# ClickHouse/libhdfs3

Measured on AMD Instinct MI355X. Metric: device-resident CRC32C GiB/s over 512 B HDFS chunks; % of HBM roofline, higher is better.
Workload: dtype u8

## Files before the change

libhdfs3_amd/csrc/crc32c_experiments.hip:

```cpp
#include "crc32c_wave.h"

namespace hdfs3crc {
namespace {

template <int BPC, bool V>
hipError_t launch_exp(const LaunchEnv &env, int variant, const ChunkLaunch &a) {
    const auto [tab, fold, grid_cap, s] = std::tie(env.tables, env.fold, env.grid_cap, env.stream);
    if constexpr (BPC > kRoundBytes) {
        if (variant == 115) return launch_r3<BPC, V, 1, true, true>(a, tab, fold, grid_cap, s);
        if (variant == 123) return launch_r3<BPC, V, 1, true>(a, tab, fold, grid_cap, s);
    }
    if constexpr (BPC <= kRoundBytes) {
        switch (variant) {
        case 92:
            return launch_wave3<BPC, V, false, true, kLabEarly>(a, tab, fold, grid_cap, s);
        case 93:
            return launch_wave3<BPC, V, false, false>(a, tab, fold, grid_cap, s);
        case 94:
            return launch_wave3<BPC, V, false, V>(a, tab, fold, grid_cap, s);
        case 95:
            return launch_wave3<BPC, V, false, true, kLabNoHold>(a, tab, fold, grid_cap, s);
        case 77:
            return launch_wave3<BPC, V, false, true, kLabNoMath>(a, tab, fold, grid_cap, s);
        case 99:
        case 100: {
            const uint64_t units = a.len / kRoundBytes;
            const uint64_t npk = variant == 99 ? 1 : 8;
            const uint64_t upp = units / npk;
            if (a.len % kRoundBytes || units % npk || (upp & (upp - 1)) || a.chunk_base) return hipErrorInvalidValue;
            ChunkLaunch p = a;
            p.npk = npk;
            p.pitch = upp * kRoundBytes;
            p.crc_pitch = upp * (kRoundBytes / BPC) * 4;
            p.last_len = uint32_t(upp * kRoundBytes);
            if (!packet_geom(p.pitch, p.last_len, npk, BPC, &p.geom)) return hipErrorInvalidValue;
            return launch_wave3<BPC, V, true, false>(p, tab, fold, grid_cap, s);
        }
        case 115:
            return launch_wave3<BPC, V, false, true, kLabPrio>(a, tab, fold, grid_cap, s);
        case 117:
            return launch_wave3<BPC, V, false, true, kLabNoPrio>(a, tab, fold, grid_cap, s);
        case 118:
            return launch_wave3<BPC, V, false, true, kLabNoStore>(a, tab, fold, grid_cap, s);
        case 119:
            return launch_wave3<BPC, V, false, true, kLabNearStore>(a, tab, fold, grid_cap, s);
        case 123:
            return launch_wave3<BPC, V, false, true>(a, tab, fold, grid_cap, s);
        case 122:
            return launch_wave3<BPC, V, false, true, kLabNoStage>(a, tab, fold, grid_cap, s);
        case 130:
            return launch_wave3<BPC, V, false, true, kLabStageWin>(a, tab, fold, grid_cap, s);
        case 157:
            return launch_wave3<BPC, V, false, true, kLabFull16>(a, tab, fold, grid_cap, s);
        case 128:
            return launch_wave3<BPC, V, false, true, kLabStorePlain>(a, tab, fold, grid_cap, s);
        case 146:
            return launch_wave3<BPC, V, false, true, kLabClock | kLabMid>(a, tab, fold, grid_cap, s);
        case 147:
            return launch_wave3<BPC, V, false, true, kLabNoTabLoad | kLabClock | kLabMid>(a, tab, fold, grid_cap, s);
        case 148:
            return launch_wave3<BPC, V, false, true, kLabNoTabLoad>(a, tab, fold, grid_cap, s);
        case 137:
            return launch_wave3<BPC, V, false, true, kLabWg1024>(a, tab, fold, grid_cap, s);
        case 162:
            return launch_wave3<BPC, V, false, true, kLabOneRound>(a, tab, fold, grid_cap, s);
        case 132:
            return launch_wave3<BPC, V, false, true, 0, 256>(a, tab, fold, grid_cap, s);
        case 134:
            return launch_wave3<BPC, V, false, true, 0, 512>(a, tab, fold, grid_cap, s);
        case 125:
            return launch_wave3<BPC, V, false, true, kLabClock>(a, tab, fold, grid_cap, s);
        case 78:
            return launch_wave3<BPC, V, false, true, kLabNoMath | kLabNoFill>(a, tab, fold, grid_cap, s);
        default: return hipErrorInvalidValue;
        }
    }
    return hipErrorInvalidValue;
}

}

hipError_t launch_experiment(const LaunchEnv &env, int variant, const ChunkLaunch &a, bool verify) {
    return dispatch_bpc<true>(a.bpc, [&](auto bpc) {
        return verify ? launch_exp<bpc(), true>(env, variant, a) : launch_exp<bpc(), false>(env, variant, a);
    });
}

void set_variant(int v) { g_variant = v; }

hipError_t lab_clock_buffer(unsigned long long *d, unsigned int cap, unsigned int *n_out) {
    unsigned int n = 0;
    hipError_t e = hipMemcpyFromSymbol(&n, HIP_SYMBOL(g_lab_clk_n), sizeof n);
    if (e != hipSuccess) return e;
    if (n_out) *n_out = n;
    const unsigned int zero = 0;
    if ((e = hipMemcpyToSymbol(HIP_SYMBOL(g_lab_clk), &d, sizeof d)) != hipSuccess) return e;
    if ((e = hipMemcpyToSymbol(HIP_SYMBOL(g_lab_clk_cap), &cap, sizeof cap)) != hipSuccess) return e;
    return hipMemcpyToSymbol(HIP_SYMBOL(g_lab_clk_n), &zero, sizeof zero);
}

hipError_t lab_wave_buffer(unsigned long long *d, unsigned int cap, unsigned int *n_out) {
    if (n_out) *n_out = g_lab_seq.exchange(0);
    hipError_t e;
    const unsigned long long *none = nullptr;
    if ((e = hipMemcpyToSymbol(HIP_SYMBOL(g_lab_wave), &none, sizeof none)) != hipSuccess) return e;
    if (!d || !cap) return hipSuccess;
    if ((e = hipMemcpyToSymbol(HIP_SYMBOL(g_lab_wave_cap), &cap, sizeof cap)) != hipSuccess) return e;
    return hipMemcpyToSymbol(HIP_SYMBOL(g_lab_wave), &d, sizeof d);
}

hipError_t launch_stream_read(const uint8_t *d, uint64_t len, uint32_t *sink, int grid,
                              hipStream_t stream, bool overlap_previous) {
    const bool nt = grid < 0;
    const dim3 g(nt ? -grid : grid), b(256);
    auto k = nt ? stream_read_kernel<true> : stream_read_kernel<false>;
    if (overlap_previous)
        hipExtLaunchKernelGGL(k, g, b, 0, stream, nullptr, nullptr, hipExtAnyOrderLaunch, d, len / 16, sink,
                              g_lab_seq++);
    else
        hipLaunchKernelGGL(k, g, b, 0, stream, d, len / 16, sink, g_lab_seq++);
    return hipGetLastError();
}

hipError_t launch_lane_read(const uint8_t *d, uint64_t len, uint32_t bpc, uint32_t *sink,
                            int grid_cap, hipStream_t stream) {
    const int variant = int(bpc >> 16);
    bpc &= 0xFFFFu;
    const uint64_t chunks = len / bpc;
    const uint64_t lanes = variant == 2 ? chunks * 8 : variant == 3 ? chunks * 4 : chunks;
    const uint64_t need = (lanes + kBlockThreads - 1) / kBlockThreads;
    const int grid = int(need < uint64_t(grid_cap) ? need : uint64_t(grid_cap));
#define LR(B, V) hipLaunchKernelGGL((lane_read_kernel<B, V>), dim3(grid), dim3(kBlockThreads), 0, stream, d, chunks, sink)
#define LRV(B)                          \
    switch (variant) {                  \
    case 0: LR(B, 0); break;            \
    case 1: LR(B, 1); break;            \
    case 2: LR(B, 2); break;            \
    case 3: LR(B, 3); break;            \
    default: LR(B, 4); break;           \
    }
    switch (bpc) {
    case 512: LRV(512); break;
    case 2048: LRV(2048); break;
    case 4096: LRV(4096); break;
    default: return hipErrorInvalidValue;
    }
#undef LRV
#undef LR
    return hipGetLastError();
}

}
```

libhdfs3_amd/csrc/crc32c_wave.h:

```cpp
#pragma once

#include "crc32c_device.h"

namespace hdfs3crc {
namespace {

constexpr int kLabEarly = 1;
constexpr int kLabNoMath = 2;
constexpr int kLabNoHold = 4;
constexpr int kLabNoFill = 8;
constexpr int kLabPrio = 16;
constexpr int kLabNoPrio = 32;
constexpr int kLabNoStore = 64;
constexpr int kLabNearStore = 128;
constexpr int kLabNoStage = 1024;
constexpr int kLabStageWin = 2048;
constexpr int kLabClock = 4096;
constexpr int kLabStorePlain = 8192;
constexpr int kLabWg1024 = 16384;
constexpr int kLabNoTabLoad = 2097152;
constexpr int kLabFull16 = 8388608;
constexpr int kLabOneRound = 4194304;
constexpr int kLabMid = 1048576;
constexpr int kStageWords = 512;
constexpr uint32_t kStageMaxRounds(int bpc) { return uint32_t(bpc / 16); }

constexpr uint32_t kPrioMinRounds = 16;

typedef __attribute__((address_space(1))) const uint32_t gcu32;
typedef __attribute__((address_space(1))) const uint8_t gcu8;
typedef __attribute__((address_space(1))) uint8_t gu8;
typedef __attribute__((address_space(1))) uint32_t gu32;
typedef __attribute__((address_space(1))) unsigned long long gu64;
typedef __attribute__((address_space(4))) const SegLaunch CSegLaunch;
typedef __attribute__((address_space(4))) const DevSegment CDevSegment;

struct WView {
    const uint8_t *p;
    uint8_t *w;
    uint64_t key;
    uint32_t nb;
};

template <int CPU>
struct BlockWalk {
    static constexpr bool kLaneView = true;
    static constexpr bool kContiguous = true;
    const uint8_t *data;
    uint8_t *words;
    uint64_t key0, first, stride;
    uint32_t K;
    const uint8_t *dummy;
    uint32_t kq = 0, kr = 0;
    __device__ __forceinline__ WView view(uint32_t k) const {
        const uint64_t u = first + uint64_t(k) * stride;
        const bool in = k < K;
        return WView{in ? data + u * kRoundBytes : dummy, in ? words + 4 * CPU * u : const_cast<uint8_t *>(dummy),
                     key0 + CPU * u, uint32_t(kRoundBytes)};
    }
};

template <int CPU>
struct PitchWalk {
    static constexpr bool kLaneView = true;
    static constexpr bool kContiguous = false;
    const uint8_t *data;
    uint8_t *words;
    uint64_t dpitch, wpitch, first, stride;
    uint32_t K;
    uint32_t upp, magic, shift, ptail, lunits, ltail, lpk;
    const uint8_t *dummy;
    __device__ __forceinline__ WView view(uint32_t k) const {
        const uint32_t u = uint32_t(first + uint64_t(k) * stride);
        const uint32_t pk = uint32_t((uint64_t(u) * magic) >> shift), r = u - pk * upp;
        const bool lastp = pk == lpk;
        const uint32_t nb = r + 1 == (lastp ? lunits : upp) ? (lastp ? ltail : ptail) : uint32_t(kRoundBytes);
        const bool in = k < K;
        return WView{in ? data + uint64_t(pk) * dpitch + uint64_t(r) * kRoundBytes : dummy,
                     in ? words + uint64_t(pk) * wpitch + 4 * CPU * r : const_cast<uint8_t *>(dummy),
                     (uint64_t(pk) << 32) | (CPU * r), in ? nb : uint32_t(kRoundBytes)};
    }
};

template <int CPU, bool UNI>
struct SegWalk {
    static constexpr bool kLaneView = false;
    static constexpr bool kContiguous = false;
    CSegLaunch *L;
    uint64_t first, stride;
    uint32_t K;
    const uint8_t *dummy;
    uint64_t c_begin = 1, c_end = 0, c_key = 0;
    uint64_t c_wlen = 0;
    const uint8_t *c_data = nullptr;
    uint8_t *c_crc = nullptr;
    uint32_t c_si = ~0u;
    static constexpr uint32_t kBpc = uint32_t(kRoundBytes / CPU);

    __device__ __forceinline__ static uint64_t wlen(uint64_t len) { return len / kBpc * kBpc; }
    __device__ __forceinline__ static uint64_t units(uint64_t len) { return (wlen(len) + kRoundBytes - 1) / kRoundBytes; }
    __device__ __forceinline__ CDevSegment *segp(uint32_t i) const {
        return L->seg ? (CDevSegment *)(L->seg) + i : L->inl + i;
    }
    __device__ __forceinline__ uint32_t seg_of(uint64_t u) const {
        if constexpr (UNI) {
            const uint32_t si = uint32_t(u) / uint32_t(L->uniform);
            return si < L->nseg ? si : L->nseg - 1;
        } else {
            uint32_t lo = 0, hi = L->nseg - 1;
            while (lo < hi) {
                const uint32_t mid = (lo + hi + 1) >> 1;
                if (rfl64(segp(mid)->unit_begin) <= u) lo = mid;
                else hi = mid - 1;
            }
            return lo;
        }
    }
    __device__ __forceinline__ WView view(uint32_t k) {
        if (k >= K) return WView{dummy, const_cast<uint8_t *>(dummy), 0, uint32_t(kRoundBytes)};
        const uint64_t u = first + uint64_t(k) * stride;
        if (u < c_begin || u >= c_end) {
            uint32_t si;
            if constexpr (UNI) {
                si = seg_of(u);
            } else {
                const uint32_t nx = c_si + 1;
                if (nx < L->nseg && u >= rfl64(segp(nx)->unit_begin) &&
                    u < rfl64(segp(nx)->unit_begin) + units(rfl64(segp(nx)->len)))
                    si = nx;
                else if (L->unit_seg)
                    si = __builtin_amdgcn_readfirstlane(
                        ((__attribute__((address_space(4))) const uint32_t *)(L->unit_seg))[u]);
                else
                    si = seg_of(u);
            }
            if (L->stride) {
                const bool lastp = si + 1 >= L->nseg;
                c_begin = uint64_t(si) * L->uniform;
                c_wlen = wlen(lastp ? L->inl[1].len : L->inl[0].len);
                c_end = c_begin + (lastp ? units(L->inl[1].len) : L->uniform);
                c_data = L->inl[0].data + uint64_t(si) * L->stride;
                c_crc = L->dense_words ? L->dense_words + 4 * CPU * c_begin : L->inl[0].crc + uint64_t(si) * L->stride;
                c_key = uint64_t(si) << 32;
            } else {
                CDevSegment *sd = segp(si);
                c_begin = rfl64(sd->unit_begin);
                c_wlen = wlen(rfl64(sd->len));
                c_end = c_begin + (c_wlen + kRoundBytes - 1) / kRoundBytes;
                c_data = reinterpret_cast<const uint8_t *>(rfl64(reinterpret_cast<uint64_t>(sd->data)));
                c_crc = L->dense_words ? L->dense_words + 4 * CPU * c_begin
                                       : reinterpret_cast<uint8_t *>(rfl64(reinterpret_cast<uint64_t>(sd->crc)));
                c_key = rfl64(sd->key_base);
            }
            c_si = si;
        }
        const uint64_t r = u - c_begin, left = c_wlen - r * kRoundBytes;
        return WView{c_data + r * kRoundBytes, c_crc + 4 * CPU * r, c_key + CPU * r,
                     left < kRoundBytes ? uint32_t(left) : uint32_t(kRoundBytes)};
    }
};

template <int BPC, bool VERIFY, bool SOLO, bool HOLD, int LAB, int TPB, class Walk>
__device__ __forceinline__ void wave_rounds(Walk &walk, uint32_t *lds, const uint32_t *__restrict__ g_tab,
                                            const uint32_t *__restrict__ g_nib, unsigned long long *result,
                                            unsigned long long *lab_mid = nullptr) {
    constexpr int G = BPC / 64;
    constexpr bool kHalfFold = G <= 32;
    constexpr bool LATE = (LAB & kLabEarly) == 0, NOMATH = (LAB & kLabNoMath) != 0;
    constexpr bool kWrong = (LAB & (kLabNoMath | kLabNoFill | kLabNoTabLoad)) != 0;
    const uint32_t lane = threadIdx.x & 63;
    const uint32_t j = lane % G;
    const uint32_t lane_off = 64 * (lane & 15) + 16 * (lane >> 4);
    const uint32_t K = walk.K;

    constexpr int kFillIters = 1024 / TPB;
    static_assert(kFillIters * TPB == 1024, "TPB divides 1024");
    uint32_t tw[kFillIters];
    u32x4 n0[kFillIters], n1[kFillIters];
#pragma unroll
    for (int f = 0; f < kFillIters; ++f) {
        const uint32_t t = threadIdx.x + f * TPB;
        if constexpr ((LAB & kLabNoTabLoad) != 0) {
            tw[f] = t * 0x9E3779B9u;
            n0[f] = u32x4{t, t ^ 1u, t ^ 2u, t ^ 3u};
            n1[f] = n0[f];
            continue;
        }
        tw[f] = g_tab[t];
        if constexpr (kHalfFold) {
            const uint32_t fk = 2 * (t >> 8) + ((t >> 3) & 1), fe = (t >> 4) & 15, fc = 4 * (t & 7);
            n0[f] = *reinterpret_cast<const u32x4 *>(g_nib + (fk * 16 + fe) * 64 + fc);
        } else {
            n0[f] = *reinterpret_cast<const u32x4 *>(g_nib + 8 * t);
            n1[f] = *reinterpret_cast<const u32x4 *>(g_nib + 8 * t + 4);
        }
    }
    WView cv0 = walk.view(0), cv1 = walk.view(1);
    __builtin_amdgcn_sched_barrier(0);
    Round a0, a1, b0, b1;
    load_round_buf<true>(a0, cv0.p, lane_off, cv0.nb);
    load_round_buf<true>(a1, cv1.p, lane_off, cv1.nb);
    __builtin_amdgcn_sched_barrier(0);
#pragma unroll
    for (int f = 0; f < kFillIters; ++f) {
        const uint32_t tt = threadIdx.x + f * TPB, slice = tt >> 8, entry = tt & 255;
        const uint32_t slot0 = ((slice >> 1) << 16 | entry << 8 | (slice & 1) << 7) / 16;
        const uint32_t w = tw[f];
        const uint32_t byte_t = (slot0 | (tt & 7)) << 4;
#pragma unroll
        for (int r = 0; r < ((LAB & kLabNoFill) ? 0 : 8); ++r)
            *reinterpret_cast<u32x4 *>(reinterpret_cast<uint8_t *>(lds) + (byte_t ^ uint32_t(16 * r))) = u32x4{w, w, w, w};
        if constexpr (kHalfFold) {
            reinterpret_cast<u32x4 *>(lds + kHalfFoldOff / 4)[tt] = n0[f];
        } else {
            u32x4 *dst = reinterpret_cast<u32x4 *>(reinterpret_cast<uint8_t *>(lds) + kFoldLdsOff) + 2 * tt;
            dst[0] = n0[f];
            dst[1] = n1[f];
        }
    }
    lds_barrier();
    if constexpr ((LAB & kLabMid) != 0) lab_mid[0] = __builtin_amdgcn_s_memrealtime();
    const Lut t(lds);
    const NibFold nf(lds);
    auto fold = [&](uint32_t x) -> uint32_t {
        if constexpr (kHalfFold) return fold_half(reinterpret_cast<const uint8_t *>(lds), x);
        return nf.apply(x);
    };
    const uint32_t woff = 4 * (lane / G);
    const uint32_t coff = (lane / G) * BPC;
    WView pv0 = walk.view(2), pv1 = walk.view(3);

    auto wrsrc = [](const WView &v) {
        return __builtin_amdgcn_make_buffer_rsrc(v.w, 0, __builtin_amdgcn_readfirstlane(v.nb / (BPC / 4)), 0x00020000);
    };
    auto want_of = [&](const WView &v) -> uint32_t {
        if constexpr (VERIFY) return __builtin_amdgcn_raw_buffer_load_b32(wrsrc(v), woff, 0, 0);
        return 0;
    };
    constexpr bool kHold = HOLD && !VERIFY && G == 8;
    constexpr bool kAddr = !Walk::kLaneView;
    auto held_store = [&](gu8 *p, uint32_t v) { *(gu32 *)p = v; };
    uint32_t line = 0;
    uint32_t hold[kHold ? 8 : 1];
    gu32 *laddr = nullptr;
    gu32 *hold_addr[kHold && kAddr ? 8 : 1];
    uint32_t nheld = 0, hold_base = 0;
    auto flush = [&]() {
#pragma unroll
        for (int i = 0; i < (kHold ? 8 : 0); ++i) {
            if (uint32_t(i) < nheld && ((LAB & kLabNoStore) == 0 || hold[i] == 0x9E3779B9u)) {
                if constexpr ((LAB & kLabNearStore) != 0 && !kAddr) {
                    *(gu32 *)((gu8 *)walk.view(0).w + 4 * lane) = hold[i];
                } else if constexpr (kAddr) {
                    if (hold_addr[i]) *hold_addr[i] = hold[i];
                } else {
                    const uint32_t kk = 8 * (hold_base + nheld - 1 - i) + (lane >> 3);
                    if (kk < K) {
                        const WView v = walk.view(kk);
                        if ((lane & 7) * BPC < v.nb) held_store((gu8 *)v.w + 4 * (lane & 7), hold[i]);
                    }
                }
            }
        }
        hold_base += nheld;
        nheld = 0;
    };
    constexpr bool kStage = !VERIFY && (LAB & kStageWords) != 0 && Walk::kContiguous && kHalfFold && TPB == 1024;
    constexpr uint32_t kCpw = 64 / G;
    constexpr uint32_t kSR = kStageMaxRounds(BPC);
    uint32_t *stage = lds + kLdsBytesWave / 4 - 4096;
    const uint32_t slot = threadIdx.x >> 6;
    auto stage_store = [&](gu8 *p, uint32_t v) {
        if constexpr ((LAB & kLabNoStore) != 0) {
            if (v != 0x9E3779B9u) return;
        }
        if constexpr (kStage && (LAB & kLabStorePlain) == 0) {
            const uint64_t wb = rfl64(reinterpret_cast<uint64_t>(walk.words));
            const __amdgpu_buffer_rsrc_t rs = __builtin_amdgcn_make_buffer_rsrc(
                reinterpret_cast<void *>(wb), 0, 0x7FFFFFFF, 0x00020000);
            __builtin_amdgcn_raw_buffer_store_b32(v, rs, uint32_t(reinterpret_cast<uint64_t>(p) - wb), 0, 1 | 2 | 16);
        } else {
            *(gu32 *)p = v;
        }
    };
    uint32_t kq_flush = 0;
    if constexpr (kStage) kq_flush = walk.kq - (walk.kr == 0 ? 1u : 0u);
    auto stage_flush = [&](uint32_t kend) {
        if constexpr (kStage) {
            if (kend % kSR == 0 && kend <= kq_flush && walk.kq != 0) {
                lds_barrier();
                const uint64_t wg_first = walk.first - slot;
#pragma unroll
                for (int p = 0; p < 4; ++p) {
                    const uint32_t t = threadIdx.x + 1024 * p, kk = t / (16 * kCpw), s = (t / kCpw) & 15,
                                   c = t % kCpw;
                    stage_store((gu8 *)walk.words +
                                    4 * kCpw * (wg_first + s + uint64_t(kend - kSR + kk) * walk.stride) + 4 * c,
                                stage[t]);
                }
                lds_barrier();
            }
        }
    };
    constexpr bool kHold64 = !VERIFY && G == 64 && Walk::kContiguous && (LAB & kLabNoHold) == 0;
    uint32_t line64 = 0;
    auto finish = [&](uint32_t k, const WView &v, uint32_t y, uint32_t want) {
        if constexpr (kHold64) {
            if (k >= K) return;
            const uint32_t yy = __builtin_amdgcn_readfirstlane(y);
            line64 = lane == (k & 63) ? yy : line64;
            if ((k & 63) == 63 || k + 1 == K) {
                const uint32_t kk = (k & ~63u) + lane;
                if (lane <= (k & 63)) held_store((gu8 *)walk.view(kk).w, line64);
            }
            return;
        }
        if constexpr (kStage) {
            if (k < K && j == 0) stage[((k % kSR) * 16 + slot) * kCpw + lane / G] = y;
            return;
        }
        if constexpr (kHold) {
            if (k >= K) return;
            const uint32_t r = k & 7;
            const uint32_t got = uint32_t(__builtin_amdgcn_ds_bpermute(int(32 * (lane & 7)), int(y)));
            const bool mine = (lane >> 3) == r;
            line = mine ? got : line;
            if constexpr (kAddr)
                laddr = mine ? ((lane & 7) * BPC < v.nb ? (gu32 *)((gu8 *)v.w + 4 * (lane & 7)) : nullptr) : laddr;
            if (r == 7 || k + 1 == K) {
#pragma unroll
                for (int i = (kHold ? 7 : 0); i > 0; --i) {
                    hold[i] = hold[i - 1];
                    if constexpr (kAddr) hold_addr[i] = hold_addr[i - 1];
                }
                hold[0] = line;
                if constexpr (kAddr) {
                    hold_addr[0] = laddr;
                    laddr = nullptr;
                }
                if (++nheld == 8) flush();
            }
            return;
        }
        if (k >= K || j != 0) return;
        const uint32_t c = y;
        if constexpr (VERIFY) {
            if ((want != c) != kWrong && coff < v.nb)
                __hip_atomic_fetch_max((gu64 *)result, ~(unsigned long long)(v.key + lane / G), __ATOMIC_RELAXED,
                                       __HIP_MEMORY_SCOPE_AGENT);
        } else {
            __builtin_amdgcn_raw_buffer_store_b32(c, wrsrc(v), woff, 0, 0);
        }
    };
    auto word = [](const Round &r, int i) -> uint32_t { return r.w[i >> 2][i & 3]; };
    auto look = [&](uint32_t x) -> Look {
        if constexpr (NOMATH) return Look{{x, 0u, 0u, 0u}};
        return lookups(t, x);
    };
    auto chains = [&](Round &c0, Round &c1, uint32_t &x0, uint32_t &x1) {
        x0 = word(c0, 0);
        x1 = word(c1, 0);
        Look l0 = look(x0), l1;
        __builtin_amdgcn_sched_barrier(0);
        if constexpr ((LAB & kLabFull16) != 0) {
#pragma unroll
            for (int i = 0; i < 16; ++i) {
                l1 = look(x1);
                __builtin_amdgcn_sched_barrier(0);
                x0 = combine(l0, i < 15 ? word(c0, i < 15 ? i + 1 : 15) : 0u);
                __builtin_amdgcn_sched_barrier(0);
                if (i < 15) l0 = look(x0);
                __builtin_amdgcn_sched_barrier(0);
                x1 = combine(l1, i < 15 ? word(c1, i < 15 ? i + 1 : 15) : 0u);
                __builtin_amdgcn_sched_barrier(0);
            }
            return;
        }
#pragma unroll
        for (int i = 0; i < 15; ++i) {
            l1 = look(x1);
            __builtin_amdgcn_sched_barrier(0);
            x0 = combine(l0, word(c0, i + 1));
            __builtin_amdgcn_sched_barrier(0);
            if (i < 14) l0 = look(x0);
            __builtin_amdgcn_sched_barrier(0);
            x1 = combine(l1, word(c1, i + 1));
            __builtin_amdgcn_sched_barrier(0);
        }
    };
    auto solo = [&](Round &c, const WView &v, uint32_t k, uint32_t w, auto id) {
        uint32_t x = word(c, 0);
        if constexpr ((LAB & kLabFull16) != 0) {
#pragma unroll
            for (int i = 0; i < 16; ++i) x = combine(look(x), i < 15 ? word(c, i < 15 ? i + 1 : 15) : 0u);
        } else {
#pragma unroll
            for (int i = 0; i < 15; ++i) x = combine(look(x), word(c, i + 1));
        }
        finish(k, v, group_xor<G>(fold(x)), w);
        if constexpr (decltype(id)::value == 0) asm volatile("; solo round 0" ::: "memory");
        else asm volatile("; solo round 1" ::: "memory");
    };
    const bool use_prio = (LAB & kLabPrio) != 0 || ((LAB & kLabNoPrio) == 0 && K >= kPrioMinRounds);
    auto prio = [&](uint32_t k) {
        if (use_prio) {
            const uint32_t left = K > k ? K - k : 0;
            if (left * 4 > 3 * K) __builtin_amdgcn_s_setprio(3);
            else if (left * 4 > 2 * K) __builtin_amdgcn_s_setprio(2);
            else if (left * 4 > K) __builtin_amdgcn_s_setprio(1);
            else __builtin_amdgcn_s_setprio(0);
        }
    };
    auto step = [&](Round &c0, Round &c1, Round &p0, Round &p1, uint32_t k) {
        prio(k);
        const uint32_t w0 = want_of(cv0), w1 = want_of(cv1);
        if constexpr (!LATE) {
            load_round_buf<true>(p0, pv0.p, lane_off, pv0.nb);
            load_round_buf<true>(p1, pv1.p, lane_off, pv1.nb);
        }
        __builtin_amdgcn_sched_barrier(0);
        regroup(c0);
        regroup(c1);
        if constexpr ((LAB & kLabMid) != 0) {
            if (k == 0) lab_mid[1] = __builtin_amdgcn_s_memrealtime();
        }
        if constexpr (LATE) {
            __builtin_amdgcn_sched_barrier(0);
            load_round_buf<true>(p0, pv0.p, lane_off, pv0.nb);
            load_round_buf<true>(p1, pv1.p, lane_off, pv1.nb);
            __builtin_amdgcn_sched_barrier(0);
        }
        uint32_t x0, x1;
        chains(c0, c1, x0, x1);
        finish(k, cv0, group_xor<G>(fold(x0)), w0);
        finish(k + 1, cv1, group_xor<G>(fold(x1)), w1);
        stage_flush(k + 2);
        __builtin_amdgcn_sched_barrier(0);
        cv0 = pv0;
        cv1 = pv1;
        pv0 = walk.view(k + 4);
        pv1 = walk.view(k + 5);
    };

    const uint32_t nr = (K + 1) & ~1u;
    if constexpr (SOLO) {
        auto last = [&](Round &c0, Round &c1, uint32_t k) {
            prio(k);
            const uint32_t w0 = want_of(cv0), w1 = want_of(cv1);
            __builtin_amdgcn_sched_barrier(0);
            regroup(c0);
            solo(c0, cv0, k, w0, std::integral_constant<int, 0>{});
            regroup(c1);
            solo(c1, cv1, k + 1, w1, std::integral_constant<int, 1>{});
            stage_flush(k + 2);
        };
        if (nr != 0) {
            const uint32_t kl = nr - 2;
            if ((kl >> 1) & 1) {
                step(a0, a1, b0, b1, 0);
                for (uint32_t k = 2; k < kl; k += 4) {
                    step(b0, b1, a0, a1, k);
                    step(a0, a1, b0, b1, k + 2);
                }
                last(b0, b1, kl);
            } else {
                for (uint32_t k = 0; k < kl; k += 4) {
                    step(a0, a1, b0, b1, k);
                    step(b0, b1, a0, a1, k + 2);
                }
                last(a0, a1, kl);
            }
        }
    } else {
        for (uint32_t k = 0; k < nr; k += 4) {
            step(a0, a1, b0, b1, k);
            if (k + 2 >= nr) break;
            step(b0, b1, a0, a1, k + 2);
        }
    }
    if constexpr (kStage) {
        lds_barrier();
        const uint64_t wg_first = walk.first - slot;
        const uint32_t wb = walk.kq ? kSR * (kq_flush / kSR) : 0u;
#pragma unroll
        for (int p = 0; p < 4; ++p) {
            const uint32_t t = threadIdx.x + 1024 * p, k = wb + t / (16 * kCpw), s = (t / kCpw) & 15, c = t % kCpw;
            const uint32_t ks = walk.kq + (wg_first + s < walk.kr ? 1u : 0u);
            if (k < ks)
                stage_store((gu8 *)walk.words + 4 * (kRoundBytes / BPC) * (wg_first + s + uint64_t(k) * walk.stride) +
                                4 * c,
                            stage[t]);
        }
    } else if constexpr (kHold) {
        flush();
    }
}

template <int BPC, bool VERIFY, int TPB = kBlockThreads>
__device__ __forceinline__ void slow_region(const uint32_t *lds, const uint8_t *sdata, uint8_t *sw, uint64_t len,
                                            uint64_t skey, int check_short_tail, unsigned long long *result) {
    constexpr int kChunksPerUnit = kRoundBytes / BPC;
    const Lut t(lds);
    const uint64_t nfull = len / BPC;
    const uint64_t first_slow = (len / kRoundBytes) * kChunksPerUnit;
    const uint64_t nslow = nfull - first_slow + (len % BPC ? 1 : 0);
    const uint64_t gtid = uint64_t(blockIdx.x) * TPB + threadIdx.x;
    const bool crc_al4 = (reinterpret_cast<uintptr_t>(sw) & 3u) == 0;
    if (gtid < nslow) {
        const uint64_t chunk = first_slow + gtid;
        const uint32_t sz = chunk < nfull ? uint32_t(BPC) : uint32_t(len % BPC);
        const uint32_t c = ~crc_run_lines(t, 0xFFFFFFFFu, sdata + chunk * BPC, sz);
        if constexpr (VERIFY) {
            if ((sz == uint32_t(BPC) || check_short_tail) && load_be32(sw + 4 * chunk, crc_al4) != c)
                atomicMax(result, ~(unsigned long long)(skey + chunk));
        } else {
            store_be32(sw + 4 * chunk, c, crc_al4);
        }
    }
}

template <int BPC, bool VERIFY, int TPB = kBlockThreads>
__device__ __forceinline__ void short_tail(const uint32_t *lds, const uint8_t *sdata, uint8_t *sw, uint64_t len,
                                           uint64_t skey, int check_short_tail, unsigned long long *result) {
    if (blockIdx.x != 0 || threadIdx.x != 0) return;
    const Lut t(lds);
    const uint64_t chunk = len / BPC;
    const bool crc_al4 = (reinterpret_cast<uintptr_t>(sw) & 3u) == 0;
    const uint32_t c = ~crc_run_lines(t, 0xFFFFFFFFu, sdata + chunk * BPC, uint32_t(len % BPC));
    if constexpr (VERIFY) {
        if (check_short_tail && load_be32(sw + 4 * chunk, crc_al4) != c)
            atomicMax(result, ~(unsigned long long)(skey + chunk));
    } else {
        store_be32(sw + 4 * chunk, c, crc_al4);
    }
}

template <int BPC, bool VERIFY, bool PITCH, bool SOLO, int LAB = 0, int TPB = kBlockThreads>
__global__ __launch_bounds__(TPB) void crc32c_wave_kernel(ChunkLaunch a, const uint32_t *__restrict__ g_tab,
                                                                    const uint32_t *__restrict__ g_nib) {
    static_assert(BPC <= kRoundBytes && BPC % 512 == 0, "one-round units");
    __shared__ __attribute__((aligned(16))) uint32_t lds[kLdsBytesWave / 4];
    constexpr int kCpu = kRoundBytes / BPC;
    constexpr int kWpb = TPB / 64;
    const uint64_t nwaves = uint64_t(gridDim.x) * kWpb;
    const uint64_t wave = uint64_t(blockIdx.x) * kWpb + __builtin_amdgcn_readfirstlane(threadIdx.x >> 6);
    uint8_t *words = VERIFY ? const_cast<uint8_t *>(a.crc_be) : a.out_be;
    const uint8_t *dummy = reinterpret_cast<const uint8_t *>(g_tab);
    constexpr bool kHold = !VERIFY && BPC == 512 && (LAB & kLabNoHold) == 0;
    const uint32_t K = a.kq + (wave < a.kr ? 1u : 0u);
    unsigned long long lab_mid[3] = {0, 0, 0};
#if HDFS3_LAB
    LabClock clk;
    if constexpr ((LAB & kLabClock) != 0) clk.start();
    if constexpr ((LAB & kLabMid) != 0) {
        asm volatile("" ::"s"(a.kq), "s"(a.kr));
        lab_mid[2] = __builtin_amdgcn_s_memrealtime();
    }
#endif
    if constexpr (PITCH) {
        const PacketGeom &g = a.geom;
        PitchWalk<kCpu> w{a.data, words, a.pitch, a.crc_pitch ? a.crc_pitch : a.pitch, wave, nwaves, K,
                          g.upp, g.magic, g.shift, g.ptail, g.lunits, g.ltail, uint32_t(a.npk - 1), dummy};
        wave_rounds<BPC, VERIFY, SOLO, kHold, LAB, TPB>(w, lds, g_tab, g_nib, a.result);
        const uint64_t lp = a.npk - 1;
        if (a.last_len % BPC)
            short_tail<BPC, VERIFY, TPB>(lds, a.data + lp * a.pitch, words + lp * w.wpitch, a.last_len, lp << 32,
                                         a.check_short_tail, a.result);
    } else {
        BlockWalk<kCpu> w{a.data, words, a.chunk_base, wave, nwaves, K, dummy, a.kq, a.kr};
        wave_rounds<BPC, VERIFY, SOLO, kHold, LAB, TPB>(w, lds, g_tab, g_nib, a.result, lab_mid);
        if (a.len % kRoundBytes)
            slow_region<BPC, VERIFY, TPB>(lds, a.data, words, a.len, a.chunk_base, a.check_short_tail, a.result);
    }
#if HDFS3_LAB
    if constexpr ((LAB & kLabClock) != 0) {
        if constexpr ((LAB & kLabMid) != 0)
            clk.end(a.lab_seq, ((lab_mid[0] - clk.r0) & 0x1FFFFF) | ((lab_mid[1] - clk.r0) & 0x1FFFFF) << 21 |
                                   ((lab_mid[2] - clk.r0) & 0x1FFFFF) << 42);
        else
            clk.end(a.lab_seq);
    }
#endif
}

template <int BPC, bool VERIFY, bool UNI, int LAB = 0, int TPB = kBlockThreads>
__global__ __launch_bounds__(TPB) void crc32c_segments_kernel(SegLaunch L, const uint32_t *__restrict__ g_tab,
                                                              const uint32_t *__restrict__ g_nib) {
    static_assert(BPC <= kRoundBytes && BPC % 512 == 0, "one-round units");
    __shared__ __attribute__((aligned(16))) uint32_t lds[kLdsBytesWave / 4];
    constexpr int kCpu = kRoundBytes / BPC;
    constexpr int kWpb = TPB / 64;
    const uint64_t nwaves = uint64_t(gridDim.x) * kWpb;
    const uint64_t wave = uint64_t(blockIdx.x) * kWpb + __builtin_amdgcn_readfirstlane(threadIdx.x >> 6);
    SegWalk<kCpu, UNI> w{(CSegLaunch *)(&L), wave, nwaves, L.kq + (wave < L.kr ? 1u : 0u),
                         reinterpret_cast<const uint8_t *>(g_tab)};
    wave_rounds<BPC, VERIFY, false, !VERIFY && BPC == 512, LAB, TPB>(w, lds, g_tab, g_nib, L.result);

    if (L.dense_words) return;
    const Lut t(lds);
    for (uint64_t si = uint64_t(threadIdx.x) * gridDim.x + blockIdx.x; si < L.nseg;
         si += uint64_t(gridDim.x) * TPB) {
        DevSegment sd;
        if (L.stride) {
            sd = L.inl[0];
            sd.data += si * L.stride;
            sd.crc += si * L.stride;
            sd.len = si + 1 < L.nseg ? L.inl[0].len : L.inl[1].len;
            sd.key_base = si << 32;
        } else {
            sd = L.seg ? L.seg[si] : L.inl[si];
        }
        if (sd.len % BPC) {
            const uint64_t c = sd.len / BPC;
            const uint32_t v = ~crc_run_lines(t, 0xFFFFFFFFu, sd.data + c * BPC, uint32_t(sd.len % BPC));
            if constexpr (VERIFY) {
                if (L.check_short_tail && load_be32(sd.crc + 4 * c, true) != v)
                    atomicMax(L.result, ~(unsigned long long)(sd.key_base + c));
            } else {
                store_be32(sd.crc + 4 * c, v, true);
            }
        }
    }
}

constexpr uint64_t kSoloTailMaxBytes = uint64_t(256) << 20;

template <int BPC, bool V, bool PITCH, bool SOLO, int LAB = 0, int TPB = kBlockThreads>
hipError_t launch_wave3(const ChunkLaunch &a, const uint32_t *tab, const uint32_t *fold, int grid_cap, hipStream_t s) {
    constexpr int G = BPC / 64;
    constexpr int set = G == 8 ? 0 : G == 16 ? 1 : G == 32 ? 2 : 3;
    const uint32_t *nib = fold + ((LAB & kLabFull16) ? kFoldAffineOldOff : kFoldAffineOff) + set * kFoldNibbleWords;
    const uint64_t units = PITCH ? (a.npk - 1) * a.geom.upp + a.geom.lunits : a.len / kRoundBytes;
    const uint64_t rpw = (LAB & kLabOneRound) != 0 && units <= 4096 ? 1 : 2;
    const uint64_t need = (units + rpw * (TPB / 64) - 1) / (rpw * (TPB / 64));
    int grid = int(need < uint64_t(grid_cap) ? need : uint64_t(grid_cap));
    if (grid < 1) grid = 1;
    const uint64_t nwaves = uint64_t(grid) * (TPB / 64);
    if (units / nwaves >= (uint64_t(1) << 32)) return hipErrorInvalidValue;
    ChunkLaunch b = a;
    if constexpr ((LAB & kLabClock) != 0) b.lab_seq = g_lab_seq++;
    b.kq = uint32_t(units / nwaves);
    b.kr = uint32_t(units % nwaves);
    if constexpr ((V || PITCH) && TPB == 1024 && (LAB & kLabWg1024) == 0) {
        constexpr int kSmall = (!V && PITCH) ? kLabNoHold : 0;
        if (units <= 4096) return launch_wave3<BPC, V, PITCH, SOLO, LAB | kSmall, 256>(a, tab, fold, grid_cap, s);
        if (units <= 16384) return launch_wave3<BPC, V, PITCH, SOLO, LAB, 512>(a, tab, fold, grid_cap, s);
    }
    if constexpr (!V && BPC <= 2048 && !PITCH && TPB == 1024 &&
                  (LAB & (kStageWords | kLabNoStage | kLabNoHold)) == 0) {
        const bool words_fit = units * uint64_t(4 * (kRoundBytes / BPC)) < (uint64_t(1) << 31);
        if (words_fit && (b.kq + (b.kr ? 1u : 0u) <= kStageMaxRounds(BPC) || BPC != 512 || (LAB & kLabStageWin) != 0))
            return launch_wave3<BPC, V, PITCH, SOLO, LAB | kStageWords, TPB>(a, tab, fold, grid_cap, s);
    }
    if (a.overlap_previous) {
        if constexpr (SOLO) {
            if (units * kRoundBytes <= kSoloTailMaxBytes) {
                hipExtLaunchKernelGGL((crc32c_wave_kernel<BPC, V, PITCH, true, LAB, TPB>), dim3(grid),
                                      dim3(TPB), 0, s, nullptr, nullptr, hipExtAnyOrderLaunch, b, tab, nib);
                return hipGetLastError();
            }
        }
        hipExtLaunchKernelGGL((crc32c_wave_kernel<BPC, V, PITCH, false, LAB, TPB>), dim3(grid),
                              dim3(TPB), 0, s, nullptr, nullptr, hipExtAnyOrderLaunch, b, tab, nib);
    } else {
        hipLaunchKernelGGL((crc32c_wave_kernel<BPC, V, PITCH, false, LAB, TPB>), dim3(grid), dim3(TPB),
                           0, s, b, tab, nib);
    }
    return hipGetLastError();
}

template <int BPC, bool V, int LAB = 0, int TPB = kBlockThreads>
hipError_t launch_segments3(const SegLaunch &in, const uint32_t *tab, const uint32_t *fold, int grid_cap,
                            hipStream_t s) {
    if constexpr (TPB == 1024) {
        if (in.units <= 4096) return launch_segments3<BPC, V, LAB, 256>(in, tab, fold, grid_cap, s);
        if (in.units <= 16384) return launch_segments3<BPC, V, LAB, 512>(in, tab, fold, grid_cap, s);
    }
    constexpr int G = BPC / 64;
    constexpr int set = G == 8 ? 0 : G == 16 ? 1 : G == 32 ? 2 : 3;
    constexpr uint64_t kWpb = TPB / 64;
    const uint32_t *nib = fold + ((LAB & kLabFull16) ? kFoldAffineOldOff : kFoldAffineOff) + set * kFoldNibbleWords;
    SegLaunch L = in;
    const uint64_t need = (L.units + 2 * kWpb - 1) / (2 * kWpb);
    const uint64_t tail_need = (L.nseg + TPB - 1) / TPB;
    uint64_t g = need > tail_need ? need : tail_need;
    g = g < uint64_t(grid_cap) ? g : uint64_t(grid_cap);
    const int grid = int(g > 0 ? g : 1);
    const uint64_t nwaves = uint64_t(grid) * kWpb;
    if (L.units / nwaves >= (uint64_t(1) << 32)) return hipErrorInvalidValue;
    L.kq = uint32_t(L.units / nwaves);
    L.kr = uint32_t(L.units % nwaves);
    if (L.uniform)
        hipLaunchKernelGGL((crc32c_segments_kernel<BPC, V, true, LAB, TPB>), dim3(grid), dim3(TPB), 0, s, L, tab, nib);
    else
        hipLaunchKernelGGL((crc32c_segments_kernel<BPC, V, false, LAB, TPB>), dim3(grid), dim3(TPB), 0, s, L, tab, nib);
    return hipGetLastError();
}

}
}
```

Baseline: 6156.

## Batch expected-CRC loads into one windowed load per G rounds in verify path

In the verify kernel, the per-round uniform buffer load of expected CRC words is replaced by one per-lane load covering a window of G rounds. Each lane holds the computed CRC for its assigned round through an inverse-ballot select, and the window is compared once when it closes. This cuts the number of small scattered reads and the waits on them in the inner loop, at the cost of extra address math, including the magic-number divide in pitched views. Large word buffers and small 256-thread launches fall back to the old path, and lab variants 170/171 are added for ablation.

```diff
diff --git a/libhdfs3_amd/csrc/crc32c_experiments.hip b/libhdfs3_amd/csrc/crc32c_experiments.hip
--- a/libhdfs3_amd/csrc/crc32c_experiments.hip
+++ b/libhdfs3_amd/csrc/crc32c_experiments.hip
@@ -70,6 +70,10 @@
             return launch_wave3<BPC, V, false, true, 0, 512>(a, tab, fold, grid_cap, s);
         case 125:
             return launch_wave3<BPC, V, false, true, kLabClock>(a, tab, fold, grid_cap, s);
+        case 170:
+            return launch_wave3<BPC, V, false, true, kLabNoWant>(a, tab, fold, grid_cap, s);
+        case 171:
+            return launch_wave3<BPC, V, false, true, kLabNoWin>(a, tab, fold, grid_cap, s);
         case 78:
             return launch_wave3<BPC, V, false, true, kLabNoMath | kLabNoFill>(a, tab, fold, grid_cap, s);
         default: return hipErrorInvalidValue;
diff --git a/libhdfs3_amd/csrc/crc32c_wave.h b/libhdfs3_amd/csrc/crc32c_wave.h
--- a/libhdfs3_amd/csrc/crc32c_wave.h
+++ b/libhdfs3_amd/csrc/crc32c_wave.h
@@ -18,6 +18,8 @@
 constexpr int kLabClock = 4096;
 constexpr int kLabStorePlain = 8192;
 constexpr int kLabWg1024 = 16384;
+constexpr int kLabNoWant = 32768;
+constexpr int kLabNoWin = 65536;
 constexpr int kLabNoTabLoad = 2097152;
 constexpr int kLabFull16 = 8388608;
 constexpr int kLabOneRound = 4194304;
@@ -57,6 +59,10 @@
         const bool in = k < K;
         return WView{in ? data + u * kRoundBytes : dummy, in ? words + 4 * CPU * u : const_cast<uint8_t *>(dummy),
                      key0 + CPU * u, uint32_t(kRoundBytes)};
+    }
+    __device__ __forceinline__ uint32_t word_off(uint32_t k, uint32_t &nb) const {
+        nb = uint32_t(kRoundBytes);
+        return 4 * CPU * (uint32_t(first) + k * uint32_t(stride));
     }
 };
 
@@ -80,6 +86,13 @@
                      in ? words + uint64_t(pk) * wpitch + 4 * CPU * r : const_cast<uint8_t *>(dummy),
                      (uint64_t(pk) << 32) | (CPU * r), in ? nb : uint32_t(kRoundBytes)};
     }
+    __device__ __forceinline__ uint32_t word_off(uint32_t k, uint32_t &nb) const {
+        const uint32_t u = uint32_t(first) + k * uint32_t(stride);
+        const uint32_t pk = uint32_t((uint64_t(u) * magic) >> shift), r = u - pk * upp;
+        const bool lastp = pk == lpk;
+        nb = r + 1 == (lastp ? lunits : upp) ? (lastp ? ltail : ptail) : uint32_t(kRoundBytes);
+        return pk * uint32_t(wpitch) + 4 * CPU * r;
+    }
 };
 
 template <int CPU, bool UNI>
@@ -195,8 +208,29 @@
             n1[f] = *reinterpret_cast<const u32x4 *>(g_nib + 8 * t + 4);
         }
     }
+    constexpr bool kWin = VERIFY && Walk::kLaneView && G <= 16 && (LAB & (kLabNoWin | kLabNoWant)) == 0;
+    uint32_t held = 0, wantw = 0;
+    auto win_lane = [&](uint32_t kb, uint32_t &off) -> bool {
+        if constexpr (kWin) {
+            uint32_t nb;
+            off = walk.word_off(kb + j, nb) + 4 * (lane / G);
+            return kb + j < K && (lane / G) * BPC < nb;
+        }
+        return false;
+    };
+    auto win_load = [&](uint32_t kb) {
+        if constexpr (kWin) {
+            uint32_t off;
+            const bool in = win_lane(kb, off);
+            const uint64_t wb = rfl64(reinterpret_cast<uint64_t>(walk.words));
+            const __amdgpu_buffer_rsrc_t rs =
+                __builtin_amdgcn_make_buffer_rsrc(reinterpret_cast<void *>(wb), 0, 0x7FFFFFFF, 0x00020000);
+            wantw = __builtin_amdgcn_raw_buffer_load_b32(rs, in ? off : 0x80000000u, 0, 0);
+        }
+    };
     WView cv0 = walk.view(0), cv1 = walk.view(1);
     __builtin_amdgcn_sched_barrier(0);
+    win_load(0);
     Round a0, a1, b0, b1;
     load_round_buf<true>(a0, cv0.p, lane_off, cv0.nb);
     load_round_buf<true>(a1, cv1.p, lane_off, cv1.nb);
@@ -234,8 +268,17 @@
         return __builtin_amdgcn_make_buffer_rsrc(v.w, 0, __builtin_amdgcn_readfirstlane(v.nb / (BPC / 4)), 0x00020000);
     };
     auto want_of = [&](const WView &v) -> uint32_t {
-        if constexpr (VERIFY) return __builtin_amdgcn_raw_buffer_load_b32(wrsrc(v), woff, 0, 0);
+        if constexpr ((LAB & kLabNoWant) != 0) return 0x9E3779B9u;
+        if constexpr (VERIFY && !kWin) return __builtin_amdgcn_raw_buffer_load_b32(wrsrc(v), woff, 0, 0);
         return 0;
+    };
+    auto win_check = [&](uint32_t kb) {
+        if constexpr (kWin) {
+            uint32_t off;
+            if (win_lane(kb, off) && (wantw != held) != kWrong)
+                __hip_atomic_fetch_max((gu64 *)result, ~(unsigned long long)(walk.view(kb + j).key + lane / G),
+                                       __ATOMIC_RELAXED, __HIP_MEMORY_SCOPE_AGENT);
+        }
     };
     constexpr bool kHold = HOLD && !VERIFY && G == 8;
     constexpr bool kAddr = !Walk::kLaneView;
@@ -342,10 +385,15 @@
             }
             return;
         }
+        if constexpr (kWin) {
+            constexpr unsigned long long kLane0 = G == 8 ? 0x0101010101010101ull : 0x0001000100010001ull;
+            held = __builtin_amdgcn_inverse_ballot_w64(kLane0 << (k & (G - 1))) ? y : held;
+            return;
+        }
         if (k >= K || j != 0) return;
         const uint32_t c = y;
         if constexpr (VERIFY) {
-            if ((want != c) != kWrong && coff < v.nb)
+            if ((want != c) != (kWrong || (LAB & kLabNoWant) != 0) && coff < v.nb)
                 __hip_atomic_fetch_max((gu64 *)result, ~(unsigned long long)(v.key + lane / G), __ATOMIC_RELAXED,
                                        __HIP_MEMORY_SCOPE_AGENT);
         } else {
@@ -411,8 +459,31 @@
             else __builtin_amdgcn_s_setprio(0);
         }
     };
+    auto win_open = [&](uint32_t k) {
+        if constexpr (kWin) {
+            if (k % G == 0 && k != 0) win_load(k);
+        }
+    };
+    auto win_open_last = [&](uint32_t k) {
+        if constexpr (kWin) {
+            const bool opens = k % G == 0 && k != 0;
+            uint32_t off;
+            const bool in = win_lane(k, off) && opens;
+            const uint64_t wb = rfl64(reinterpret_cast<uint64_t>(walk.words));
+            const __amdgpu_buffer_rsrc_t rs =
+                __builtin_amdgcn_make_buffer_rsrc(reinterpret_cast<void *>(wb), 0, 0x7FFFFFFF, 0x00020000);
+            const uint32_t w = __builtin_amdgcn_raw_buffer_load_b32(rs, in ? off : 0x80000000u, 0, 0);
+            wantw = opens ? w : wantw;
+        }
+    };
+    auto win_close = [&](uint32_t kend) {
+        if constexpr (kWin) {
+            if (kend % G == 0) win_check(kend - G);
+        }
+    };
     auto step = [&](Round &c0, Round &c1, Round &p0, Round &p1, uint32_t k) {
         prio(k);
+        if constexpr (!LATE) win_open(k);
         const uint32_t w0 = want_of(cv0), w1 = want_of(cv1);
         if constexpr (!LATE) {
             load_round_buf<true>(p0, pv0.p, lane_off, pv0.nb);
@@ -426,6 +497,7 @@
         }
         if constexpr (LATE) {
             __builtin_amdgcn_sched_barrier(0);
+            win_open(k);
             load_round_buf<true>(p0, pv0.p, lane_off, pv0.nb);
             load_round_buf<true>(p1, pv1.p, lane_off, pv1.nb);
             __builtin_amdgcn_sched_barrier(0);
@@ -434,6 +506,7 @@
         chains(c0, c1, x0, x1);
         finish(k, cv0, group_xor<G>(fold(x0)), w0);
         finish(k + 1, cv1, group_xor<G>(fold(x1)), w1);
+        win_close(k + 2);
         stage_flush(k + 2);
         __builtin_amdgcn_sched_barrier(0);
         cv0 = pv0;
@@ -446,12 +519,14 @@
     if constexpr (SOLO) {
         auto last = [&](Round &c0, Round &c1, uint32_t k) {
             prio(k);
+            win_open_last(k);
             const uint32_t w0 = want_of(cv0), w1 = want_of(cv1);
             __builtin_amdgcn_sched_barrier(0);
             regroup(c0);
             solo(c0, cv0, k, w0, std::integral_constant<int, 0>{});
             regroup(c1);
             solo(c1, cv1, k + 1, w1, std::integral_constant<int, 1>{});
+            win_close(k + 2);
             stage_flush(k + 2);
         };
         if (nr != 0) {
@@ -477,6 +552,9 @@
             if (k + 2 >= nr) break;
             step(b0, b1, a0, a1, k + 2);
         }
+    }
+    if constexpr (kWin) {
+        if (nr % G != 0) win_check(nr - nr % G);
     }
     if constexpr (kStage) {
         lds_barrier();
@@ -652,6 +730,12 @@
         if (words_fit && (b.kq + (b.kr ? 1u : 0u) <= kStageMaxRounds(BPC) || BPC != 512 || (LAB & kLabStageWin) != 0))
             return launch_wave3<BPC, V, PITCH, SOLO, LAB | kStageWords, TPB>(a, tab, fold, grid_cap, s);
     }
+    if constexpr (V && G <= 16 && (LAB & (kLabNoWin | kLabNoWant)) == 0) {
+        const uint64_t wbytes = PITCH ? a.npk * (a.crc_pitch ? a.crc_pitch : a.pitch)
+                                      : units * uint64_t(4 * (kRoundBytes / BPC));
+        if (wbytes >= (uint64_t(1) << 31) || (TPB == 256 && !a.overlap_previous))
+            return launch_wave3<BPC, V, PITCH, SOLO, LAB | kLabNoWin, TPB>(a, tab, fold, grid_cap, s);
+    }
     if (a.overlap_previous) {
         if constexpr (SOLO) {
             if (units * kRoundBytes <= kSoloTailMaxBytes) {
```

New measurement: 6189 (median of 5 runs). About the same (+0.5%).
